# intel/intel-extension-for-transformers

Hardware: AMD Instinct MI355X
Metric: decode tokens/sec + achieved HBM GB/s, Llama-2-7B int4 WOQ, batch=1 (higher is better)
Workload: dtype int4 weights x fp32 activations (3 int8 limbs on i8 MFMA, exact int32 tile sums, fp32 across tiles); 1 GPU; Llama-2-7B int4 sym group_size=128 fp16 scales, batch=1 greedy decode, prompt 32, lm_head fp16 unquantised, KV fp16; global_batch=1, parallelism=single GPU, hipgraph=True

## Files before the change

include/woq_hip_experimental.h:

```cpp
#ifndef WOQ_HIP_EXPERIMENTAL_H_
#define WOQ_HIP_EXPERIMENTAL_H_

#include "woq_hip.h"

#ifdef __cplusplus
extern "C" {
#endif

WOQ_API int woq_engine_set_attn_chunk(woq_engine* e, int chunk);
WOQ_API int woq_engine_attn_chunk(woq_engine* e);
WOQ_API int woq_engine_time_gemv(woq_engine* e, int reps, void* stream, float* total_ms, double* bytes_per_pass,
                                 int* launches_per_pass);
WOQ_API int woq_engine_time_gemv_mask(woq_engine* e, int mask, int reps, void* stream, float* total_ms,
                                      double* bytes_per_pass, int* launches_per_pass);
WOQ_API int woq_engine_time_twin(woq_engine* e, int mode, int reps, void* stream, float* total_ms);
WOQ_API int woq_engine_set_time_eager(woq_engine* e, int on);
WOQ_API int woq_engine_time_prefill_gemm(woq_engine* e, int layer, int n_rows, int reps, void* stream, float* gemm_ms,
                                         float* call_ms);
WOQ_API int woq_gemm_form_log(int* forms, int cap);
WOQ_API int woq_probe_rope_append(void* qkv, int n_seq, int T, int start, int heads, int kv_heads, int head_dim,
                                  const float* cos_dev, const float* sin_dev, void* kcache, void* vcache, int kv_dtype,
                                  size_t seq_stride_elems, void* stream);
WOQ_API int woq_probe_attn_prefill(const void* qkv, int n_seq, int T, int start, int heads, int kv_heads, int head_dim,
                                   const void* kcache, const void* vcache, int kv_dtype, size_t seq_stride_elems,
                                   void* out, int window, void* stream);
WOQ_API int woq_probe_attn_decode(const float* qkv, void* kcache, void* vcache, int kv_dtype, const int32_t* pos_dev,
                                  const float* cos_dev, const float* sin_dev, int heads, int kv_heads, int head_dim,
                                  int max_ctx, int window, int splits, int grouped, int merge, int chunk_fixed,
                                  float* out, void* stream);
WOQ_API int woq_probe_sample(const float* logits, int vocab, uint32_t* seen, const woq_sampler_config* cfg,
                             const float* u_or_null, const int32_t* pos_dev, int32_t* token_out, uint32_t* philox_out4,
                             int* status, void* stream);

#ifdef __cplusplus
}
#endif
#endif
```

intel_extension_for_transformers_amd/_lib.py:

```python
import ctypes
import os

_HERE = os.path.dirname(os.path.abspath(__file__))
LIB_PATH = os.environ.get("WOQ_HIP_LIB") or os.path.join(_HERE, "libwoq_hip.so")

F32, BF16, F16, FP8_E4M3 = 0, 1, 2, 3
W_INT4_CLIP, W_INT8, W_NF4, W_FP4_E2M1, W_FP4_E2M1_BNB, W_INT3_CLIP, W_INT2_CLIP = 0, 1, 2, 3, 4, 5, 6
W_FP8_E4M3, W_FP8_E5M2 = 7, 8
S_FP8_E8M0 = 4
FLAG_SCALE_E8M0 = 4
C_FP32, C_BF16, C_INT8, C_FP16 = 0, 1, 2, 3
HEADER_BYTES = 256

WEIGHT_TYPES = {"int4_clip": W_INT4_CLIP, "int4": W_INT4_CLIP, "int8": W_INT8, "nf4": W_NF4, "fp4_e2m1": W_FP4_E2M1,
                "fp4": W_FP4_E2M1, "fp4_e2m1_bnb": W_FP4_E2M1_BNB, "int3_clip": W_INT3_CLIP, "int2_clip": W_INT2_CLIP,
                "fp8_e4m3": W_FP8_E4M3, "fp8": W_FP8_E4M3, "fp8_e5m2": W_FP8_E5M2}
SCALE_TYPES = {"fp32": F32, "bf16": BF16, "fp16": F16, "fp8_e8m0": S_FP8_E8M0}
COMPUTE_TYPES = {"fp32": C_FP32, "bf16": C_BF16, "int8": C_INT8, "fp16": C_FP16}
SCALE_NAMES = {F32: "fp32", BF16: "bf16", F16: "fp16"}
COMPUTE_NAMES = {v: k for k, v in COMPUTE_TYPES.items()}
WEIGHT_NAMES = {W_INT4_CLIP: "int4_clip", W_INT8: "int8", W_NF4: "nf4", W_FP4_E2M1: "fp4_e2m1",
                W_FP4_E2M1_BNB: "fp4_e2m1_bnb", W_FP8_E4M3: "fp8_e4m3", W_FP8_E5M2: "fp8_e5m2"}


class BlobHeader(ctypes.Structure):

    _fields_ = [
        ("magic", ctypes.c_uint32), ("version", ctypes.c_uint32), ("total_bytes", ctypes.c_uint64),
        ("K", ctypes.c_int32), ("N", ctypes.c_int32), ("group", ctypes.c_int32), ("Kpad", ctypes.c_int32),
        ("Npad", ctypes.c_int32), ("n_groups", ctypes.c_int32),
        ("weight_type", ctypes.c_uint32), ("scale_type", ctypes.c_uint32), ("compute_type", ctypes.c_uint32),
        ("flags", ctypes.c_uint32), ("scale_mode", ctypes.c_uint32), ("narrow_bits", ctypes.c_uint32),
        ("off_q", ctypes.c_uint64), ("off_scale", ctypes.c_uint64), ("off_zp", ctypes.c_uint64),
        ("off_shuffle", ctypes.c_uint64), ("pad", ctypes.c_uint8 * (HEADER_BYTES - 96)),
    ]


assert ctypes.sizeof(BlobHeader) == HEADER_BYTES


class EngineConfig(ctypes.Structure):
    _fields_ = [(n, ctypes.c_int32) for n in ("hidden", "inter", "heads", "kv_heads", "head_dim", "layers", "vocab",
                                              "max_ctx")] + [("rms_eps", ctypes.c_float), ("rope_theta", ctypes.c_float),
                                                             ("tp_rank", ctypes.c_int32), ("tp_size", ctypes.c_int32),
                                                             ("kv_dtype", ctypes.c_int32),
                                                             ("reserved", ctypes.c_int32 * 3)]


class LayerWeights(ctypes.Structure):
    _fields_ = [("qkv_blob", ctypes.c_void_p), ("o_blob", ctypes.c_void_p), ("gate_up_blob", ctypes.c_void_p),
                ("down_blob", ctypes.c_void_p), ("ln1", ctypes.c_void_p), ("ln2", ctypes.c_void_p),
                ("qkv_hdr", BlobHeader), ("o_hdr", BlobHeader), ("gate_up_hdr", BlobHeader), ("down_hdr", BlobHeader)]


class SamplerConfig(ctypes.Structure):

    _fields_ = [("do_sample", ctypes.c_int32), ("top_k", ctypes.c_int32), ("temperature", ctypes.c_float),
                ("top_p", ctypes.c_float), ("repetition_penalty", ctypes.c_float), ("seed_lo", ctypes.c_uint32),
                ("seed_hi", ctypes.c_uint32), ("reserved", ctypes.c_uint32)]


ALLREDUCE_FN = ctypes.CFUNCTYPE(ctypes.c_int, ctypes.c_void_p, ctypes.c_void_p, ctypes.c_size_t, ctypes.c_void_p)

EXPORTS = [
    "woq_last_error", "woq_abi_version", "woq_device_count", "woq_packed_weight_size",
    "woq_repack_quantized_weight", "woq_quantize_to_packed_weight", "woq_dequantize_packed_weight",
    "woq_read_header", "woq_blob_extract", "woq_linear", "woq_rmsnorm", "woq_rope", "woq_silu_mul", "woq_gelu",
    "woq_engine_create", "woq_engine_destroy", "woq_engine_set_layer", "woq_engine_set_head",
    "woq_engine_bind_io", "woq_engine_token_ptr", "woq_engine_pos_ptr", "woq_engine_logits_ptr", "woq_engine_hidden_ptr",
    "woq_engine_step", "woq_engine_capture", "woq_engine_replay", "woq_engine_steps", "woq_engine_set_allreduce",
    "woq_engine_phase", "woq_engine_prefill", "woq_engine_prefill_logits_ptr", "woq_engine_kv_cache_ptr",
    "woq_engine_set_attn_splits", "woq_engine_attn_splits", "woq_engine_set_attn_grouped", "woq_engine_attn_grouped",
    "woq_engine_set_tp_options", "woq_engine_set_fuse_attn", "woq_engine_fuse_attn", "woq_engine_status",
    "woq_engine_clear_status", "woq_comm_create", "woq_comm_handle", "woq_comm_connect", "woq_comm_allreduce_f32",
    "woq_comm_status", "woq_comm_set_timeout_ms", "woq_comm_destroy", "woq_engine_set_comm", "woq_set_workspace",
    "woq_engine_uses_xq", "woq_engine_token_log_ptr", "woq_table_digit_planes",
    "woq_engine_set_sampler", "woq_engine_sampler_seen", "woq_engine_sampler_seen_ptr",
]
EXPERIMENTAL_EXPORTS = [
    "woq_engine_set_attn_chunk", "woq_engine_attn_chunk", "woq_engine_time_gemv", "woq_engine_time_gemv_mask",
    "woq_engine_time_twin", "woq_engine_set_time_eager", "woq_engine_time_prefill_gemm", "woq_gemm_form_log",
    "woq_probe_rope_append", "woq_probe_attn_prefill", "woq_probe_attn_decode", "woq_probe_sample",
]
GEMM_FORM_FRAG, GEMM_FORM_SPLITK, GEMM_FORM_FP32, GEMM_FORM_HANDSCHED = 1, 2, 4, 8
GEMM_FORM_RING, GEMM_FORM_TALL, GEMM_FORM_RAW = 16, 32, 64

_lib = None


def lib():
    global _lib
    if _lib is not None:
        return _lib
    if not os.path.exists(LIB_PATH):
        raise RuntimeError(
            "QBits: %s not found. Build it with `python -c 'import __graft_entry__ as g; g.build()'` "
            "(hipcc --offload-arch=gfx950); there is no CPU fallback for the MI355X path." % LIB_PATH)
    L = ctypes.CDLL(LIB_PATH)
    vp, ci, cs, cf = ctypes.c_void_p, ctypes.c_int, ctypes.c_size_t, ctypes.c_float
    L.woq_last_error.restype = ctypes.c_char_p
    L.woq_packed_weight_size.restype = cs
    L.woq_packed_weight_size.argtypes = [ci] * 7
    L.woq_table_digit_planes.restype = ci
    L.woq_table_digit_planes.argtypes = [ci, ci, vp, vp]
    L.woq_repack_quantized_weight.argtypes = [vp, vp, vp, vp, ci, ci, ci, ci, ci, ci, vp, cs, vp]
    L.woq_quantize_to_packed_weight.argtypes = [vp, ci, ci, ci, ci, ci, ci, ci, ci, vp, cs, vp]
    L.woq_dequantize_packed_weight.argtypes = [vp, ctypes.POINTER(BlobHeader), vp, ci, vp]
    L.woq_read_header.argtypes = [vp, ctypes.POINTER(BlobHeader), vp]
    L.woq_blob_extract.argtypes = [vp, ctypes.POINTER(BlobHeader), ci, vp, vp]
    L.woq_linear.argtypes = [vp, ci, ci, vp, ctypes.POINTER(BlobHeader), vp, vp, ci, ci, ci, vp]
    L.woq_rmsnorm.argtypes = [vp, ci, vp, cf, ci, ci, vp, ci, vp]
    L.woq_rope.argtypes = [vp, ci, vp, vp, vp, ci, ci, ci, vp]
    L.woq_silu_mul.argtypes = [vp, vp, ci, cs, vp, vp]
    L.woq_gelu.argtypes = [vp, ci, cs, ci, vp, vp]
    L.woq_engine_create.argtypes = [ctypes.POINTER(EngineConfig), ctypes.POINTER(vp)]
    L.woq_engine_destroy.argtypes = [vp]
    L.woq_engine_destroy.restype = None
    L.woq_engine_set_layer.argtypes = [vp, ci, ctypes.POINTER(LayerWeights)]
    L.woq_engine_set_head.argtypes = [vp, vp, ci, vp, vp, ci, vp, vp]
    for f in ("woq_engine_token_ptr", "woq_engine_pos_ptr", "woq_engine_logits_ptr", "woq_engine_hidden_ptr"):
        getattr(L, f).restype = vp
        getattr(L, f).argtypes = [vp]
    L.woq_engine_bind_io.argtypes = [vp, vp, vp, vp, vp]
    L.woq_engine_step.argtypes = [vp, ci, vp]
    L.woq_engine_capture.argtypes = [vp, ci, vp]
    L.woq_engine_replay.argtypes = [vp, ci, vp]
    L.woq_engine_steps.argtypes = [vp, ci, ci, vp]
    L.woq_engine_set_time_eager.argtypes = [vp, ci]
    L.woq_engine_set_allreduce.argtypes = [vp, ALLREDUCE_FN, vp]
    L.woq_engine_phase.argtypes = [vp, ci, ci, ci, vp]
    L.woq_engine_prefill.argtypes = [vp, vp, ci, ci, ci, ci, vp]
    L.woq_engine_prefill_logits_ptr.restype = vp
    L.woq_engine_prefill_logits_ptr.argtypes = [vp]
    L.woq_engine_set_attn_splits.argtypes = [vp, ci]
    L.woq_engine_attn_splits.argtypes = [vp]
    L.woq_engine_set_attn_grouped.argtypes = [vp, ci]
    L.woq_engine_attn_grouped.argtypes = [vp]
    L.woq_engine_set_attn_chunk.argtypes = [vp, ci]
    L.woq_engine_attn_chunk.argtypes = [vp]
    L.woq_engine_set_fuse_attn.argtypes = [vp, ci]
    L.woq_engine_fuse_attn.argtypes = [vp]
    L.woq_engine_status.argtypes = [vp, vp]
    L.woq_engine_clear_status.argtypes = [vp, vp]
    L.woq_engine_kv_cache_ptr.restype = vp
    L.woq_engine_kv_cache_ptr.argtypes = [vp, ci]
    L.woq_engine_time_gemv.argtypes = [vp, ci, vp, ctypes.POINTER(cf), ctypes.POINTER(ctypes.c_double),
                                       ctypes.POINTER(ci)]
    L.woq_engine_time_gemv_mask.argtypes = [vp, ci, ci, vp, ctypes.POINTER(cf), ctypes.POINTER(ctypes.c_double),
                                            ctypes.POINTER(ci)]
    L.woq_engine_time_twin.argtypes = [vp, ci, ci, vp, ctypes.POINTER(cf)]
    L.woq_engine_set_tp_options.argtypes = [vp, ci, ci]
    L.woq_engine_time_prefill_gemm.argtypes = [vp, ci, ci, ci, vp, ctypes.POINTER(cf), ctypes.POINTER(cf)]
    L.woq_gemm_form_log.argtypes = [ctypes.POINTER(ci), ci]
    L.woq_probe_rope_append.argtypes = [vp, ci, ci, ci, ci, ci, ci, vp, vp, vp, vp, ci, cs, vp]
    L.woq_probe_attn_prefill.argtypes = [vp, ci, ci, ci, ci, ci, ci, vp, vp, ci, cs, vp, ci, vp]
    L.woq_probe_attn_decode.argtypes = [vp, vp, vp, ci, vp, vp, vp] + [ci] * 9 + [vp, vp]
    L.woq_comm_create.argtypes = [ci, ci, cs, ctypes.POINTER(vp)]
    L.woq_comm_handle.argtypes = [vp, vp, cs]
    L.woq_comm_connect.argtypes = [vp, vp, ctypes.POINTER(ci)]
    L.woq_comm_allreduce_f32.argtypes = [vp, vp, cs, vp]
    L.woq_comm_status.argtypes = [vp, vp, ctypes.POINTER(ci)]
    L.woq_comm_set_timeout_ms.argtypes = [vp, ci]
    L.woq_comm_destroy.argtypes = [vp]
    L.woq_comm_destroy.restype = None
    L.woq_engine_set_comm.argtypes = [vp, vp, ci]
    L.woq_set_workspace.argtypes = [vp, cs]
    L.woq_engine_uses_xq.argtypes = [vp]
    L.woq_engine_token_log_ptr.restype = vp
    L.woq_engine_token_log_ptr.argtypes = [vp]
    L.woq_engine_set_sampler.argtypes = [vp, ctypes.POINTER(SamplerConfig)]
    L.woq_engine_sampler_seen.argtypes = [vp, vp, ci, ci, vp]
    L.woq_engine_sampler_seen_ptr.restype = vp
    L.woq_engine_sampler_seen_ptr.argtypes = [vp]
    L.woq_probe_sample.argtypes = [vp, ci, vp, ctypes.POINTER(SamplerConfig), vp, vp, vp, vp, vp, vp]
    _lib = L
    return L


def gemm_form_log():
    buf = (ctypes.c_int * 64)()
    n = lib().woq_gemm_form_log(buf, 64)
    return list(buf[:min(n, 64)])


def _ptr(t):
    return ctypes.c_void_p(t.data_ptr())


def probe_rope_append(qkv, n_seq, T, start, heads, kv_heads, head_dim, cos, sin, kcache, vcache, kv_dtype, seq_stride):
    rc = lib().woq_probe_rope_append(_ptr(qkv), n_seq, T, start, heads, kv_heads, head_dim, _ptr(cos), _ptr(sin),
                                     _ptr(kcache), _ptr(vcache), kv_dtype, seq_stride, stream_ptr())
    if rc != 0:
        raise RuntimeError(lib().woq_last_error().decode())


def probe_attn_prefill(qkv, n_seq, T, start, heads, kv_heads, head_dim, kcache, vcache, kv_dtype, seq_stride, out,
                       window):
    rc = lib().woq_probe_attn_prefill(_ptr(qkv), n_seq, T, start, heads, kv_heads, head_dim, _ptr(kcache), _ptr(vcache),
                                      kv_dtype, seq_stride, _ptr(out), window, stream_ptr())
    if rc != 0:
        raise RuntimeError(lib().woq_last_error().decode())


def probe_attn_decode(qkv, kcache, vcache, kv_dtype, pos, cos, sin, heads, kv_heads, head_dim, max_ctx, window, splits,
                      grouped, merge, chunk_fixed, out):
    rc = lib().woq_probe_attn_decode(_ptr(qkv), _ptr(kcache), _ptr(vcache), kv_dtype, _ptr(pos), _ptr(cos), _ptr(sin),
                                     heads, kv_heads, head_dim, max_ctx, window, splits, grouped, merge, chunk_fixed,
                                     _ptr(out), stream_ptr())
    if rc != 0:
        raise RuntimeError(lib().woq_last_error().decode())


def sampler_config(do_sample=False, temperature=1.0, top_k=0, top_p=1.0, repetition_penalty=1.0, seed=0):
    seed = int(seed) & 0xFFFFFFFFFFFFFFFF
    return SamplerConfig(do_sample=int(bool(do_sample)), top_k=int(top_k or 0),
                         temperature=float(1.0 if temperature is None else temperature),
                         top_p=float(1.0 if top_p is None else top_p),
                         repetition_penalty=float(1.0 if repetition_penalty is None else repetition_penalty),
                         seed_lo=seed & 0xFFFFFFFF, seed_hi=seed >> 32, reserved=0)


def probe_sample(logits, seen, cfg, pos, token_out, u=None, philox_out=None, status=None):
    opt = lambda t: _ptr(t) if t is not None else None
    rc = lib().woq_probe_sample(_ptr(logits), int(logits.numel()), _ptr(seen), ctypes.byref(cfg), opt(u), _ptr(pos),
                                _ptr(token_out), opt(philox_out), opt(status), stream_ptr())
    if rc != 0:
        raise RuntimeError(lib().woq_last_error().decode())


def check(rc):
    if rc != 0:
        raise RuntimeError(lib().woq_last_error().decode())


def require_gpu():
    import torch

    if not torch.cuda.is_available() or lib().woq_device_count() == 0:
        raise RuntimeError("QBits: no MI355X/HIP device visible; the gfx950 WOQ path has no CPU fallback")


def torch_dtype_code(dt):
    import torch

    if dt == torch.float32:
        return F32
    if dt == torch.bfloat16:
        return BF16
    if dt == torch.float16:
        return F16
    raise RuntimeError("QBits: unsupported qbits data type.")


def stream_ptr():
    import torch

    return ctypes.c_void_p(torch.cuda.current_stream().cuda_stream)
```

intel_extension_for_transformers_amd/csrc/woq_host.h:

```cpp
#pragma once
#include "woq_comm_dev.h"
#include "woq_launch.h"
#include "woq_xq.h"

namespace woq {
struct AttnA2A;
struct AttnMerge;
struct LutArgs;

int launch_gemv_from_header(const void* act, int act_dtype, int lda, const void* blob, const woq_blob_header& h,
                            const float* bias, void* out, int out_dtype, int ldo, int M, const float* norm_w,
                            float eps, const float* residual, int ld_res, int epi, int nt, hipStream_t st);
int launch_gemv_fp8(const void* act, int act_dtype, int lda, const void* hi_blob, const woq_blob_header& hi,
                    const void* lo_q, uint32_t fp8_type, const float* bias, void* out, int out_dtype, int ldo, int M,
                    hipStream_t st);
int launch_gemv_fp8_engine(const float* act, int lda, const void* hi_blob, const woq_blob_header& hi, const void* lo_q,
                           uint32_t fp8_type, float* out, int ldo, const float* norm_w, float eps, const float* residual,
                           int ld_res, int epi, float* gu_tmp, hipStream_t st);

int lut_args_for(uint32_t weight_type, uint32_t compute_type, LutArgs& L);
bool gemv_tile_geometry(int tiles_k, int cb, int smode, int& nw, int& tpw);
int gemv_tile_k_chunks(int tiles_k, int cb, int smode, bool chainable);
int gemv_tile_max_rows(const void* act, int act_dtype, int lda, const woq_blob_header& h, const float* norm_w,
                       int epi, int out_dtype);
int launch_gemv_tile(const void* act, int act_dtype, int lda, int M, const void* blob, const woq_blob_header& h,
                     const float* bias, void* out, int out_dtype, int ldo, const float* norm_w, float eps,
                     const float* residual, int ld_res, int epi, hipStream_t st);

bool gemv_fp8_mfma_supported(const void* act, int act_dtype, int lda, const woq_blob_header& hi);
int launch_gemv_fp8_mfma(const void* act, int act_dtype, int lda, int M, const void* hi_blob, const woq_blob_header& hi,
                         const void* lo_q, uint32_t fp8_type, const float* bias, void* out, int out_dtype, int ldo,
                         hipStream_t st, const float* norm_w = nullptr, float eps = 0.f, const float* residual = nullptr,
                         int ld_res = 0);
void launch_silu_mul_tiles(const float* gu, int inter, float* act, hipStream_t st);

bool gemv_xq_supported(const woq_blob_header& h, int epi);
int launch_gemv_xq(const XqPtrs& xin, const void* blob, const woq_blob_header& h, const float* bias, float* out,
                   const float* ssq_in, float eps, const float* residual, int epi, const XqPtrs& xo,
                   const float* next_norm_w, float* ssq_out, hipStream_t st, const CommDev* tp);
int launch_gemv_twin(const void* blob, const woq_blob_header& h, int epi, int mode, unsigned int* sink, hipStream_t st);

bool gemv_xq_attn_supported(const woq_blob_header& h, int heads, int kv_heads, int head_dim, int kv_dtype, int max_ctx,
                            int window, int splits);
int launch_gemv_xq_attn(const XqPtrs& xin, const void* blob, const woq_blob_header& h, unsigned long long* qkv_g,
                        const float* ssq_in, float eps, const unsigned int* seq, int layer, int* status, void* kcache,
                        void* vcache, int kv_dtype, const int32_t* pos, const float* cs, const float* sn, int heads,
                        int kv_heads, int max_ctx, int window, float* attn_out, const XqPtrs& xq_attn, hipStream_t st,
                        int splits = 1, unsigned long long* part_g = nullptr);

void launch_embed(const void* embed, int dtype, const int32_t* token, int hidden, float* out, const float* norm_w,
                  const XqPtrs& xo, float* ssq_out, unsigned int* step_seq, int32_t* pos, int max_ctx, int* status,
                  hipStream_t st);
int launch_attn_decode(const float* qkv, void* kcache, void* vcache, int kv_dtype, const int32_t* pos,
                       const float* cs, const float* sn, int heads, int kv_heads, int D, int max_ctx, int window,
                       float* out, int splits, int grouped, float* part, const XqPtrs& xo, hipStream_t st,
                       unsigned int* merge_counters, int chunk_fixed, const AttnA2A* a2a_grouped = nullptr,
                       const unsigned int* seq = nullptr, int layer = 0);
void launch_attn_combine(const float* part, int heads, int D, int splits, float* out, const XqPtrs& xo,
                         hipStream_t st);
void launch_lm_head(const float* hidden_in, const float* norm_w, float eps, const void* W, int w_dtype, int hidden,
                    int vocab, float* logits, float* pmax, int32_t* pidx, hipStream_t st);
void launch_argmax(const float* logits, int vocab, int32_t* token, int32_t* pos, hipStream_t st);
void launch_argmax_pairs(const float* pmax, const int32_t* pidx, int n, int32_t* token, int32_t* pos, int32_t* log,
                         hipStream_t st);
void launch_argmax_embed(const float* pmax, const int32_t* pidx, int n, int32_t* token, int32_t* pos, int32_t* log,
                         const void* embed, int dtype, int hidden, float* out, const float* norm_w, const XqPtrs& xo,
                         float* ssq_out, unsigned int* step_seq, int max_ctx, int* status, hipStream_t st);

void launch_sample(const float* logits, int vocab, uint32_t* seen, const woq_sampler_config* cfg_dev, const float* u_dev,
                   int32_t* token, int32_t* pos_advance, const int32_t* pos_fixed, int32_t* log, uint32_t* philox_out,
                   int* status, hipStream_t st);
void launch_sampler_seen(uint32_t* seen, int vocab, const int32_t* tokens, int n, hipStream_t st);
void launch_sampler_config_store(const woq_sampler_config& cfg, woq_sampler_config* dst, hipStream_t st);
const char* sampler_config_problem(const woq_sampler_config& cfg);

void launch_embed_rows(const void* embed, int dtype, const int32_t* tokens, int M, int hidden, float* out,
                       hipStream_t st);
int launch_rope_append(_Float16* qkv, int n_seq, int T, int start, int heads, int kv_heads, int HD, const float* cs,
                       const float* sn, void* kcache, void* vcache, int kv_dtype, size_t seq_stride_elems,
                       hipStream_t st);
int launch_attn_prefill(const _Float16* qkv, int n_seq, int T, int start, int heads, int kv_heads, int HD,
                        const void* kcache, const void* vcache, int kv_dtype, size_t seq_stride_elems, _Float16* out,
                        int window, hipStream_t st);
void launch_gather_last(const float* h, int n_seq, int T, int hidden, float* dst, hipStream_t st);
bool launch_attn_decode_mfma(const float* qkv, void* kcache, void* vcache, int kv_dtype, const int32_t* pos,
                             const float* cs, const float* sn, int heads, int kv_heads, int D, int window, int splits,
                             float* part, int chunk_fixed, int max_ctx, const AttnMerge& mg, hipStream_t st);
int attn_decode_mfma_slots(int kv_dtype, int rep);

size_t gemm_f16_workspace_bytes_blob(int M, const woq_blob_header& h, int planes);
int launch_gemm_f16(const void* act, int act_dtype, int lda, const void* blob, const woq_blob_header& h,
                    const float* bias, void* out, int out_dtype, int ldo, int M, const float* norm_w, float eps,
                    const float* residual, int ld_res, int epi, void* ws, int fp32_class, hipStream_t st,
                    const void* fp8_lo = nullptr, uint32_t fp8_type = 0, size_t ws_bytes = 0);
void set_gemm_time_events(hipEvent_t before, hipEvent_t after);
}

size_t woq_comm_max_elems(woq_comm* c);
int woq_comm_launch_allreduce(woq_comm* c, float* buf, size_t n, hipStream_t st);
int woq_comm_launch_allreduce_ex(woq_comm* c, float* buf, size_t n, int pushed, const float* norm_w,
                                 const woq::XqPtrs& xo, float* ssq_out, hipStream_t st);
const woq::CommDev* woq_comm_dev_ptr(woq_comm* c);
int woq_comm_launch_greedy(woq_comm* c, const float* pmax, const int32_t* pidx, int n, int vocab_offset,
                           int32_t* token, int32_t* pos, int32_t* log, hipStream_t st);
```

intel_extension_for_transformers_amd/csrc/woq_ops.hip:

```cpp
#include "woq_attn_decode.h"
#include "woq_device.h"
#include "woq_host.h"
#include "woq_xq.h"
#include "../../include/woq_hip_experimental.h"

namespace woq {

__global__ __launch_bounds__(256) void rmsnorm_kernel(const void* __restrict__ x, int dtype,
                                                      const float* __restrict__ w, float eps, int d,
                                                      void* __restrict__ out, int out_dtype) {
  __shared__ float part[4];
  const size_t row = blockIdx.x;
  const int tid = threadIdx.x;
  float ss = 0.f;
  for (int i = tid; i < d; i += 256) {
    float v = load_f32(x, row * d + i, dtype);
    ss = fmaf(v, v, ss);
  }
  ss = wave_sum(ss);
  if ((tid & 63) == 0) part[tid >> 6] = ss;
  __syncthreads();
  const float tot = part[0] + part[1] + part[2] + part[3];
  const float inv = 1.0f / sqrtf(tot / (float)d + eps);
  for (int i = tid; i < d; i += 256) {
    float v = load_f32(x, row * d + i, dtype);
    store_f32(out, row * d + i, out_dtype, v * inv * w[i]);
  }
}

__global__ void rope_kernel(void* __restrict__ x, int dtype, const int32_t* __restrict__ pos,
                            const float* __restrict__ cs, const float* __restrict__ sn, int heads, int D,
                            size_t total_pairs) {
  size_t idx = (size_t)blockIdx.x * blockDim.x + threadIdx.x;
  if (idx >= total_pairs) return;
  const int half = D >> 1;
  const int i = (int)(idx % half);
  const size_t th = idx / half;
  const int t = (int)(th / heads);
  const int p = pos[t];
  const float c = cs[(size_t)p * half + i], s = sn[(size_t)p * half + i];
  const size_t base = th * D;
  const float a = load_f32(x, base + i, dtype), b = load_f32(x, base + i + half, dtype);
  store_f32(x, base + i, dtype, a * c - b * s);
  store_f32(x, base + i + half, dtype, b * c + a * s);
}

__global__ void silu_mul_kernel(const void* __restrict__ g, const void* __restrict__ u, int dtype, size_t n,
                                void* __restrict__ out) {
  size_t idx = (size_t)blockIdx.x * blockDim.x + threadIdx.x;
  const size_t stride = (size_t)gridDim.x * blockDim.x;
  for (; idx < n; idx += stride) {
    const float a = load_f32(g, idx, dtype), b = load_f32(u, idx, dtype);
    store_f32(out, idx, dtype, a / (1.0f + expf(-a)) * b);
  }
}

__global__ void gelu_kernel(const void* __restrict__ x, int dtype, size_t n, int approximate,
                            void* __restrict__ out) {
  size_t idx = (size_t)blockIdx.x * blockDim.x + threadIdx.x;
  const size_t stride = (size_t)gridDim.x * blockDim.x;
  for (; idx < n; idx += stride) {
    const float v = load_f32(x, idx, dtype);
    float r;
    if (approximate)
      r = 0.5f * v * (1.0f + tanhf(0.7978845608028654f * (v + 0.044715f * v * v * v)));
    else
      r = 0.5f * v * (1.0f + erff(v * 0.7071067811865476f));
    store_f32(out, idx, dtype, r);
  }
}


__global__ void embed_kernel(const void* __restrict__ embed, int dtype, const int32_t* __restrict__ token, int hidden,
                             float* __restrict__ out, const float* __restrict__ norm_w, XqPtrs xo,
                             float* __restrict__ ssq_out, unsigned int* __restrict__ step_seq,
                             int32_t* __restrict__ pos, int max_ctx, int* __restrict__ status) {
  const int i = blockIdx.x * blockDim.x + threadIdx.x;
  if (i == 0) {
    if (step_seq != nullptr) step_seq[0] = step_seq[0] + 1u;
    if (pos != nullptr && pos[0] >= max_ctx) {
      pos[0] = max_ctx - 1;
      if (status != nullptr) atomicOr(status, 2);
    }
  }
  if (i < hidden) {
    const float v = load_f32(embed, (size_t)token[0] * hidden + i, dtype);
    out[i] = v;
    if (xo.limbs != nullptr) {
      const float ss = row16_sum(v * v);
      if ((i & 15) == 0) ssq_out[i >> 4] = ss;
      xq_emit16(v * norm_w[i], xo, i >> 4, i & 15);
    }
  }
}

__global__ __launch_bounds__(256) void argmax_embed_kernel(const float* __restrict__ pmax, const int32_t* __restrict__ pidx,
                                                           int n_pairs, int32_t* __restrict__ token,
                                                           int32_t* __restrict__ pos, int32_t* __restrict__ log,
                                                           const void* __restrict__ embed, int dtype, int hidden,
                                                           float* __restrict__ out, const float* __restrict__ norm_w,
                                                           XqPtrs xo, float* __restrict__ ssq_out,
                                                           unsigned int* __restrict__ step_seq, int max_ctx,
                                                           int* __restrict__ status) {
  __shared__ float bv[4];
  __shared__ int bi[4];
  const int tid = threadIdx.x, lane = tid & 63, wid = tid >> 6;
  float best = -INFINITY;
  int idx = 0x7fffffff;
  for (int i = tid; i < n_pairs; i += 256) {
    const float v = pmax[i];
    const int ci = pidx[i];
    if (v > best || (v == best && ci < idx)) best = v, idx = ci;
  }
#pragma unroll
  for (int o = 32; o > 0; o >>= 1) {
    const float ov = __shfl_xor(best, o, 64);
    const int oi = __shfl_xor(idx, o, 64);
    if (ov > best || (ov == best && oi < idx)) best = ov, idx = oi;
  }
  if (lane == 0) bv[wid] = best, bi[wid] = idx;
  __syncthreads();
  best = bv[0], idx = bi[0];
#pragma unroll
  for (int w = 1; w < 4; ++w)
    if (bv[w] > best || (bv[w] == best && bi[w] < idx)) best = bv[w], idx = bi[w];
  const bool no_winner = idx < 0 || (size_t)idx >= (size_t)n_pairs * 16;
  if (no_winner) idx = 0;
  if (blockIdx.x == 0 && tid == 0) {
    if (no_winner && status != nullptr) atomicOr(status, 4);
    token[0] = idx;
    int p = pos[0];
    if (log != nullptr) log[p] = idx;
    p += 1;
    if (step_seq != nullptr) step_seq[0] = step_seq[0] + 1u;
    if (p >= max_ctx) {
      p = max_ctx - 1;
      if (status != nullptr) atomicOr(status, 2);
    }
    pos[0] = p;
  }
  const int i = blockIdx.x * 256 + tid;
  if (i < hidden) {
    const float v = load_f32(embed, (size_t)idx * hidden + i, dtype);
    out[i] = v;
    if (xo.limbs != nullptr) {
      const float ss = row16_sum(v * v);
      if ((i & 15) == 0) ssq_out[i >> 4] = ss;
      xq_emit16(v * norm_w[i], xo, i >> 4, i & 15);
    }
  }
}

template <typename KV, int HD, bool SPLIT>
__global__ __launch_bounds__(256) void attn_decode_kernel(const float* __restrict__ qkv, KV* __restrict__ kcache,
                                                          KV* __restrict__ vcache, const int32_t* __restrict__ pos_p,
                                                          const float* __restrict__ cs, const float* __restrict__ sn,
                                                          int hk, int window, int spw,
                                                          float* __restrict__ out, XqPtrs xo, AttnMerge mg) {
  extern __shared__ __attribute__((aligned(16))) float sm[];
  const int heads = hk & 0xffff, kv_heads = hk >> 16;
  const int bx = (int)blockIdx.x;
  const int h = (heads & 7) == 0 ? (bx & 7) * (heads >> 3) + (bx >> 3) : bx;
  attn_decode_body<KV, HD, SPLIT>(sm, h, (int)blockIdx.y, (int)gridDim.y, AttnPlain{qkv}, kcache, vcache, pos_p, cs,
                                  sn, heads, kv_heads, window, spw, out, xo);
  if constexpr (SPLIT) {
    if (mg.counter != nullptr) attn_slices_merge<HD, 1>(out, heads, h, 1, (int)gridDim.y, mg.counter + h, mg, sm);
  }
}

template <int HD>
__global__ __launch_bounds__(256) void attn_combine_kernel(const float* __restrict__ part, int ns,
                                                          float* __restrict__ out, XqPtrs xo) {
  __shared__ float ms[64], wl[64], wsc[64], red[256];
  constexpr int GROUPS = 256 / HD;
  constexpr int PER = ATTN_MAX_SLICES / GROUPS;
  const int h = blockIdx.x, tid = threadIdx.x;
  const int d = tid % HD, grp = tid / HD;
  const float* p = part + (size_t)h * ATTN_MAX_SLICES * HD;
  const float* pml = part + (size_t)gridDim.x * ATTN_MAX_SLICES * HD + (size_t)h * ATTN_MAX_SLICES * 2;
  const int si = min(tid, ns - 1);
  const float m_r = pml[si * 2], l_r = pml[si * 2 + 1];
  float v[PER];
#pragma unroll
  for (int u = 0; u < PER; ++u) v[u] = p[(size_t)min(grp + u * GROUPS, ns - 1) * HD + d];
  if (tid < ns) ms[tid] = m_r, wl[tid] = l_r;
  __syncthreads();
  float m = -INFINITY;
  for (int s = 0; s < ns; ++s) m = fmaxf(m, ms[s]);
  if (tid < ns) {
    const float w = ms[tid] == -INFINITY ? 0.f : __expf(ms[tid] - m);
    wsc[tid] = w;
    wl[tid] *= w;
  }
  __syncthreads();
  float l = 0.f;
  for (int s = 0; s < ns; ++s) l += wl[s];
  float o = 0.f;
#pragma unroll
  for (int u = 0; u < PER; ++u) {
    const int s = grp + u * GROUPS;
    if (s < ns) o = fmaf(v[u], wsc[s], o);
  }
  red[tid] = o;
  __syncthreads();
  if (grp == 0) {
    float t = 0.f;
#pragma unroll
    for (int g2 = 0; g2 < GROUPS; ++g2) t += red[g2 * HD + d];
    out[(size_t)h * HD + d] = t / l;
    if (xo.limbs != nullptr) xq_emit16(t / l, xo, (h * HD + d) >> 4, d & 15);
  }
}

__global__ __launch_bounds__(256) void lm_head_kernel(const float* __restrict__ hidden_in,
                                                      const float* __restrict__ norm_w, float eps,
                                                      const void* __restrict__ W, int w_dtype, int hidden, int vocab,
                                                      float* __restrict__ logits, float* __restrict__ pmax,
                                                      int32_t* __restrict__ pidx) {
  extern __shared__ __attribute__((aligned(16))) float sm[];
  float* xs = sm;
  __shared__ float part[4];
  __shared__ float bestv[4];
  __shared__ int besti[4];
  const int tid = threadIdx.x, lane = tid & 63, wid = tid >> 6;
  float wbest = -INFINITY;
  int wbi = 0x7fffffff;
  typedef unsigned int u32x4 __attribute__((ext_vector_type(4)));
  float ss = 0.f;
  for (int i = tid; i < hidden; i += 256) {
    const float v = hidden_in[i];
    xs[i] = v;
    ss = fmaf(v, v, ss);
  }
  ss = wave_sum(ss);
  if (lane == 0) part[wid] = ss;
  __syncthreads();
  const float inv = 1.0f / sqrtf((part[0] + part[1] + part[2] + part[3]) / (float)hidden + eps);
  for (int i = tid; i < hidden; i += 256) xs[i] = xs[i] * inv * norm_w[i];
  __syncthreads();
  const int rows_per_wg = 16;
  auto consume = [&](const u32x4& raw, int k0, float& acc) {
    const uint32_t rr[4] = {raw.x, raw.y, raw.z, raw.w};
#pragma unroll
    for (int j = 0; j < 4; ++j) {
      float lo, hi;
      if (w_dtype == WOQ_BF16) {
        lo = bf16_bits_to_f32(rr[j] & 0xffff);
        hi = bf16_bits_to_f32(rr[j] >> 16);
      } else {
        lo = f16_bits_to_f32(rr[j] & 0xffff);
        hi = f16_bits_to_f32(rr[j] >> 16);
      }
      acc = fmaf(lo, xs[k0 + 2 * j], acc);
      acc = fmaf(hi, xs[k0 + 2 * j + 1], acc);
    }
  };
  auto finish = [&](int v, float acc) {
    acc = wave_sum(acc);
    if (lane == 0) logits[v] = acc;
    if (acc > wbest) {
      wbest = acc;
      wbi = v;
    }
  };
  for (int r = wid; r < rows_per_wg; r += 4) {
    const int v = blockIdx.x * rows_per_wg + r;
    if (v >= vocab) break;
    const uint16_t* wr = (const uint16_t*)W + (size_t)v * hidden;
    float acc = 0.f;
    for (int k0 = lane * 8; k0 < hidden; k0 += 512) consume(__builtin_nontemporal_load((const u32x4*)(wr + k0)), k0, acc);
    finish(v, acc);
  }
  if (pmax) {
    if (lane == 0) {
      bestv[wid] = wbest;
      besti[wid] = wbi;
    }
    __syncthreads();
    if (tid == 0) {
      float b = bestv[0];
      int bi = besti[0];
      for (int w = 1; w < 4; ++w)
        if (bestv[w] > b || (bestv[w] == b && besti[w] < bi)) {
          b = bestv[w];
          bi = besti[w];
        }
      pmax[blockIdx.x] = b;
      pidx[blockIdx.x] = bi;
    }
  }
}

__global__ __launch_bounds__(1024) void argmax_kernel(const float* __restrict__ logits, const int32_t* __restrict__ cand,
                                                      int vocab, int32_t* __restrict__ token,
                                                      int32_t* __restrict__ pos, int32_t* __restrict__ log) {
  __shared__ float bv[16];
  __shared__ int bi[16];
  const int tid = threadIdx.x, lane = tid & 63, wid = tid >> 6;
  float best = -INFINITY;
  int idx = 0x7fffffff;
  for (int i = tid; i < vocab; i += 1024) {
    const float v = logits[i];
    const int ci = cand ? cand[i] : i;
    if (v > best || (v == best && ci < idx)) {
      best = v;
      idx = ci;
    }
  }
#pragma unroll
  for (int o = 32; o > 0; o >>= 1) {
    const float ov = __shfl_xor(best, o, 64);
    const int oi = __shfl_xor(idx, o, 64);
    if (ov > best || (ov == best && oi < idx)) {
      best = ov;
      idx = oi;
    }
  }
  if (lane == 0) {
    bv[wid] = best;
    bi[wid] = idx;
  }
  __syncthreads();
  if (tid == 0) {
    for (int w = 1; w < 16; ++w)
      if (bv[w] > best || (bv[w] == best && bi[w] < idx)) {
        best = bv[w];
        idx = bi[w];
      }
    token[0] = idx;
    if (log != nullptr) log[pos[0]] = idx;
    pos[0] = pos[0] + 1;
  }
}

void launch_embed(const void* embed, int dtype, const int32_t* token, int hidden, float* out, const float* norm_w,
                  const XqPtrs& xo, float* ssq_out, unsigned int* step_seq, int32_t* pos, int max_ctx, int* status,
                  hipStream_t st) {
  hipLaunchKernelGGL(embed_kernel, dim3((hidden + 255) / 256), dim3(256), 0, st, embed, dtype, token, hidden, out,
                     norm_w, xo, ssq_out, step_seq, pos, max_ctx, status);
}

template <typename KV, int HD>
static int launch_attn_t(const float* qkv, void* kcache, void* vcache, const int32_t* pos, const float* cs,
                         const float* sn, int heads, int kv_heads, int max_ctx, int window, float* out, int splits,
                         float* part, const XqPtrs& xo, unsigned int* merge_counters, hipStream_t st) {
  const int reach = window > 0 ? min(window, max_ctx) : max_ctx;
  const int span = splits > 1 ? ((((reach + splits - 1) / splits) + 63) & ~63) + 64 : reach;
  const int spw = attn_dec_spw(span);
  const size_t lds = attn_dec_lds_floats(HD, span) * 4;
  if (lds > 160 * 1024) return woq::fail("QBits: max_ctx too large for the decode attention (raise attn_splits)");
  if (splits > 1) {
    auto k = attn_decode_kernel<KV, HD, true>;
    static bool once = false;
    if (!once) {
      hipFuncSetAttribute((const void*)k, hipFuncAttributeMaxDynamicSharedMemorySize, 160 * 1024);
      once = true;
    }
    const AttnMerge mg{merge_counters, out, xo};
    hipLaunchKernelGGL(k, dim3(heads, splits), dim3(256), lds, st, qkv, (KV*)kcache, (KV*)vcache, pos, cs, sn,
                       heads | (kv_heads << 16), window, spw, part, XqPtrs{nullptr, nullptr, nullptr}, mg);
    if (merge_counters == nullptr)
      hipLaunchKernelGGL(attn_combine_kernel<HD>, dim3(heads), dim3(256), 0, st, part, splits, out, xo);
    return 0;
  }
  auto k = attn_decode_kernel<KV, HD, false>;
  static bool once = false;
  if (!once) {
    hipFuncSetAttribute((const void*)k, hipFuncAttributeMaxDynamicSharedMemorySize, 160 * 1024);
    once = true;
  }
  hipLaunchKernelGGL(k, dim3(heads), dim3(256), lds, st, qkv, (KV*)kcache, (KV*)vcache, pos, cs, sn,
                     heads | (kv_heads << 16), window, spw, out, xo,
                     AttnMerge{nullptr, nullptr, XqPtrs{nullptr, nullptr, nullptr}});
  return 0;
}

int launch_attn_decode(const float* qkv, void* kcache, void* vcache, int kv_dtype, const int32_t* pos,
                       const float* cs, const float* sn, int heads, int kv_heads, int D, int max_ctx, int window,
                       float* out, int splits, int grouped, float* part, const XqPtrs& xo, hipStream_t st,
                       unsigned int* merge_counters, int chunk_fixed, const AttnA2A* a2a_grouped, const unsigned int* seq,
                       int layer) {
  if (D != 64 && D != 128) return woq::fail("QBits: attention head_dim must be 64 or 128");
  if (splits > ATTN_MAX_SLICES) return woq::fail("QBits: at most 64 context slices");
  AttnMerge mg{merge_counters, out, xo};
  const bool a2a = grouped && a2a_grouped != nullptr && merge_counters == nullptr && splits <= 32;
  if (a2a) mg.part_g = a2a_grouped->part_g, mg.seq = seq, mg.layer = layer, mg.status = a2a_grouped->status;
  if (grouped && launch_attn_decode_mfma(qkv, kcache, vcache, kv_dtype, pos, cs, sn, heads, kv_heads, D, window, splits,
                                          part, chunk_fixed, max_ctx, mg, st)) {
    if (merge_counters == nullptr && !a2a) launch_attn_combine(part, heads, D, splits, out, xo, st);
    return 0;
  }
#define WOQ_ATTN_DEC(T)                                                                                              \
  return D == 128 ? launch_attn_t<T, 128>(qkv, kcache, vcache, pos, cs, sn, heads, kv_heads, max_ctx, window, out,   \
                                          splits, part, xo, merge_counters, st)                                     \
                  : launch_attn_t<T, 64>(qkv, kcache, vcache, pos, cs, sn, heads, kv_heads, max_ctx, window, out,    \
                                         splits, part, xo, merge_counters, st);
  if (kv_dtype == WOQ_F16) { WOQ_ATTN_DEC(_Float16) }
  if (kv_dtype == WOQ_FP8_E4M3) { WOQ_ATTN_DEC(Fp8) }
  WOQ_ATTN_DEC(__bf16)
#undef WOQ_ATTN_DEC
}

void launch_attn_combine(const float* part, int heads, int D, int splits, float* out, const XqPtrs& xo,
                         hipStream_t st) {
  if (D == 128)
    hipLaunchKernelGGL(attn_combine_kernel<128>, dim3(heads), dim3(256), 0, st, part, splits, out, xo);
  else
    hipLaunchKernelGGL(attn_combine_kernel<64>, dim3(heads), dim3(256), 0, st, part, splits, out, xo);
}

void launch_lm_head(const float* hidden_in, const float* norm_w, float eps, const void* W, int w_dtype, int hidden,
                    int vocab, float* logits, float* pmax, int32_t* pidx, hipStream_t st) {
  hipLaunchKernelGGL(lm_head_kernel, dim3((vocab + 15) / 16), dim3(256), (size_t)hidden * 4, st, hidden_in, norm_w,
                     eps, W, w_dtype, hidden, vocab, logits, pmax, pidx);
}

void launch_argmax(const float* logits, int vocab, int32_t* token, int32_t* pos, hipStream_t st) {
  hipLaunchKernelGGL(argmax_kernel, dim3(1), dim3(1024), 0, st, logits, (const int32_t*)nullptr, vocab, token, pos,
                     (int32_t*)nullptr);
}

void launch_argmax_pairs(const float* pmax, const int32_t* pidx, int n, int32_t* token, int32_t* pos, int32_t* log,
                         hipStream_t st) {
  hipLaunchKernelGGL(argmax_kernel, dim3(1), dim3(1024), 0, st, pmax, pidx, n, token, pos, log);
}

void launch_argmax_embed(const float* pmax, const int32_t* pidx, int n, int32_t* token, int32_t* pos, int32_t* log,
                         const void* embed, int dtype, int hidden, float* out, const float* norm_w, const XqPtrs& xo,
                         float* ssq_out, unsigned int* step_seq, int max_ctx, int* status, hipStream_t st) {
  hipLaunchKernelGGL(argmax_embed_kernel, dim3((hidden + 255) / 256), dim3(256), 0, st, pmax, pidx, n, token, pos, log,
                     embed, dtype, hidden, out, norm_w, xo, ssq_out, step_seq, max_ctx, status);
}

}

using namespace woq;

extern "C" {

int woq_rmsnorm(const void* x_dev, int dtype, const float* weight_dev, float eps, int rows, int d, void* out_dev,
                int out_dtype, void* stream) {
  WOQ_TRY
  WOQ_CHECK(rows >= 0 && d > 0, "QBits: bad rmsnorm shape");
  if (rows == 0) return 0;
  hipLaunchKernelGGL(rmsnorm_kernel, dim3(rows), dim3(256), 0, (hipStream_t)stream, x_dev, dtype, weight_dev, eps, d,
                     out_dev, out_dtype);
  WOQ_HIP(hipGetLastError());
  WOQ_END
}

int woq_rope(void* x_dev, int dtype, const int32_t* pos_dev, const float* cos_dev, const float* sin_dev, int tokens,
             int heads, int D, void* stream) {
  WOQ_TRY
  WOQ_CHECK((D & 1) == 0, "QBits: rope head_dim must be even");
  size_t total = (size_t)tokens * heads * (D / 2);
  if (total == 0) return 0;
  hipLaunchKernelGGL(rope_kernel, dim3((unsigned)((total + 255) / 256)), dim3(256), 0, (hipStream_t)stream, x_dev,
                     dtype, pos_dev, cos_dev, sin_dev, heads, D, total);
  WOQ_HIP(hipGetLastError());
  WOQ_END
}

int woq_silu_mul(const void* gate_dev, const void* up_dev, int dtype, size_t n, void* out_dev, void* stream) {
  WOQ_TRY
  if (n == 0) return 0;
  unsigned blocks = (unsigned)std::min<size_t>((n + 255) / 256, 2048);
  hipLaunchKernelGGL(silu_mul_kernel, dim3(blocks), dim3(256), 0, (hipStream_t)stream, gate_dev, up_dev, dtype, n,
                     out_dev);
  WOQ_HIP(hipGetLastError());
  WOQ_END
}

int woq_gelu(const void* x_dev, int dtype, size_t n, int approximate, void* out_dev, void* stream) {
  WOQ_TRY
  if (n == 0) return 0;
  unsigned blocks = (unsigned)std::min<size_t>((n + 255) / 256, 2048);
  hipLaunchKernelGGL(gelu_kernel, dim3(blocks), dim3(256), 0, (hipStream_t)stream, x_dev, dtype, n, approximate,
                     out_dev);
  WOQ_HIP(hipGetLastError());
  WOQ_END
}

WOQ_API int woq_probe_attn_decode(const float* qkv, void* kcache, void* vcache, int kv_dtype, const int32_t* pos_dev,
                                  const float* cos_dev, const float* sin_dev, int heads, int kv_heads, int head_dim,
                                  int max_ctx, int window, int splits, int grouped, int merge, int chunk_fixed,
                                  float* out, void* stream) {
  WOQ_TRY
  WOQ_CHECK(heads > 0 && kv_heads > 0 && heads % kv_heads == 0 && max_ctx > 0 && window >= 0 && splits >= 1,
            "QBits: bad attention shape");
  WOQ_CHECK(merge == 0 || merge == 1, "QBits: merge must be 0 (combine launch) or 1 (last-arriver counters)");
  const hipStream_t st = (hipStream_t)stream;
  const size_t part_bytes = (size_t)heads * ATTN_MAX_SLICES * (head_dim + 2) * sizeof(float);
  float* part = nullptr;
  unsigned int* counters = nullptr;
  WOQ_HIP(hipMallocAsync((void**)&part, part_bytes, st));
  if (merge) {
    if (hipMallocAsync((void**)&counters, (size_t)heads * sizeof(unsigned int), st) != hipSuccess ||
        hipMemsetAsync(counters, 0, (size_t)heads * sizeof(unsigned int), st) != hipSuccess) {
      if (counters) hipFreeAsync(counters, st);
      hipFreeAsync(part, st);
      return woq::fail("QBits: could not allocate the attention merge counters");
    }
  }
  const int rc = launch_attn_decode(qkv, kcache, vcache, kv_dtype, pos_dev, cos_dev, sin_dev, heads, kv_heads, head_dim,
                                    max_ctx, window, out, splits, grouped, part, XqPtrs{nullptr, nullptr, nullptr}, st,
                                    counters, chunk_fixed, nullptr, nullptr, 0);
  const hipError_t le = hipGetLastError();
  if (counters) hipFreeAsync(counters, st);
  hipFreeAsync(part, st);
  if (rc) return rc;
  WOQ_HIP(le);
  WOQ_END
}

}
```

Baseline: 693.6 tokens/s.

## Add streamed lm_head kernel with double-buffered nontemporal row loads

Adds a templated lm_head kernel for fixed hidden sizes. Each wave streams one fp16 or bf16 vocab row at a time using 128-bit nontemporal loads, double-buffering the next row while the current one is multiplied. RMSNorm is fused into the block prologue and reduced with permlane/DPP wave sums, and the kernel keeps the per-block argmax pair output. It is dispatched by default for hidden 4096, and a probe API can force the generic or streamed form; the cost is extra specialised code paths and fixed launch bounds/occupancy per shape.

```diff
diff --git a/include/woq_hip_experimental.h b/include/woq_hip_experimental.h
--- a/include/woq_hip_experimental.h
+++ b/include/woq_hip_experimental.h
@@ -31,6 +31,8 @@
 WOQ_API int woq_probe_sample(const float* logits, int vocab, uint32_t* seen, const woq_sampler_config* cfg,
                              const float* u_or_null, const int32_t* pos_dev, int32_t* token_out, uint32_t* philox_out4,
                              int* status, void* stream);
+WOQ_API int woq_probe_lm_head(const float* hidden_in, const float* norm_w, float eps, const void* W, int w_dtype,
+                              int hidden, int vocab, float* logits, float* pmax, int32_t* pidx, int form, void* stream);
 
 #ifdef __cplusplus
 }
diff --git a/intel_extension_for_transformers_amd/_lib.py b/intel_extension_for_transformers_amd/_lib.py
--- a/intel_extension_for_transformers_amd/_lib.py
+++ b/intel_extension_for_transformers_amd/_lib.py
@@ -81,6 +81,7 @@
     "woq_engine_set_attn_chunk", "woq_engine_attn_chunk", "woq_engine_time_gemv", "woq_engine_time_gemv_mask",
     "woq_engine_time_twin", "woq_engine_set_time_eager", "woq_engine_time_prefill_gemm", "woq_gemm_form_log",
     "woq_probe_rope_append", "woq_probe_attn_prefill", "woq_probe_attn_decode", "woq_probe_sample",
+    "woq_probe_lm_head",
 ]
 GEMM_FORM_FRAG, GEMM_FORM_SPLITK, GEMM_FORM_FP32, GEMM_FORM_HANDSCHED = 1, 2, 4, 8
 GEMM_FORM_RING, GEMM_FORM_TALL, GEMM_FORM_RAW = 16, 32, 64
@@ -173,6 +174,7 @@
     L.woq_engine_sampler_seen_ptr.restype = vp
     L.woq_engine_sampler_seen_ptr.argtypes = [vp]
     L.woq_probe_sample.argtypes = [vp, ci, vp, ctypes.POINTER(SamplerConfig), vp, vp, vp, vp, vp, vp]
+    L.woq_probe_lm_head.argtypes = [vp, vp, cf, vp, ci, ci, ci, vp, vp, vp, ci, vp]
     _lib = L
     return L
 
@@ -228,6 +230,17 @@
         raise RuntimeError(lib().woq_last_error().decode())
 
 
+LM_HEAD_DISPATCH, LM_HEAD_GENERIC, LM_HEAD_STREAM = 0, 1, 2
+
+
+def probe_lm_head(hidden_in, norm_w, eps, W, hidden, vocab, logits, pmax=None, pidx=None, form=LM_HEAD_DISPATCH):
+    opt = lambda t: _ptr(t) if t is not None else None
+    rc = lib().woq_probe_lm_head(_ptr(hidden_in), _ptr(norm_w), eps, _ptr(W), torch_dtype_code(W.dtype), hidden, vocab,
+                                 _ptr(logits), opt(pmax), opt(pidx), form, stream_ptr())
+    if rc != 0:
+        raise RuntimeError(lib().woq_last_error().decode())
+
+
 def check(rc):
     if rc != 0:
         raise RuntimeError(lib().woq_last_error().decode())
diff --git a/intel_extension_for_transformers_amd/csrc/woq_host.h b/intel_extension_for_transformers_amd/csrc/woq_host.h
--- a/intel_extension_for_transformers_amd/csrc/woq_host.h
+++ b/intel_extension_for_transformers_amd/csrc/woq_host.h
@@ -59,7 +59,7 @@
 void launch_attn_combine(const float* part, int heads, int D, int splits, float* out, const XqPtrs& xo,
                          hipStream_t st);
 void launch_lm_head(const float* hidden_in, const float* norm_w, float eps, const void* W, int w_dtype, int hidden,
-                    int vocab, float* logits, float* pmax, int32_t* pidx, hipStream_t st);
+                    int vocab, float* logits, float* pmax, int32_t* pidx, hipStream_t st, int form = 0);
 void launch_argmax(const float* logits, int vocab, int32_t* token, int32_t* pos, hipStream_t st);
 void launch_argmax_pairs(const float* pmax, const int32_t* pidx, int n, int32_t* token, int32_t* pos, int32_t* log,
                          hipStream_t st);
diff --git a/intel_extension_for_transformers_amd/csrc/woq_lm_head.h b/intel_extension_for_transformers_amd/csrc/woq_lm_head.h
--- /dev/null
+++ b/intel_extension_for_transformers_amd/csrc/woq_lm_head.h
@@ -0,0 +1,135 @@
+#pragma once
+#include "woq_device.h"
+
+namespace woq {
+
+__device__ __forceinline__ float wave_sum_xor_valu(float v) {
+  float a = v, b = v;
+  asm volatile("v_nop\n\tv_nop\n\tv_permlane32_swap_b32 %0, %1" : "+v"(a), "+v"(b));
+  v = a + b;
+  a = v, b = v;
+  asm volatile("v_nop\n\tv_nop\n\tv_permlane16_swap_b32 %0, %1" : "+v"(a), "+v"(b));
+  v = a + b;
+  v += WOQ_DPP_F32(v, 0x128);
+  v += WOQ_DPP_F32(v, 0x124);
+  v += WOQ_DPP_F32(v, 0x4E);
+  v += WOQ_DPP_F32(v, 0xB1);
+  return v;
+}
+
+constexpr bool lm_head_stream_shape(int hidden) {
+  return hidden == 512 || hidden == 1024 || hidden == 4096 || hidden == 8192;
+}
+
+template <int C, int U, int OCC, bool BF16, bool MATH>
+__global__ __launch_bounds__(256, OCC) void lm_head_stream_kernel(const float* __restrict__ hidden_in,
+                                                                  const float* __restrict__ norm_w, float eps,
+                                                                  const void* __restrict__ W, int hidden, int vocab,
+                                                                  float* __restrict__ logits, float* __restrict__ pmax,
+                                                                  int32_t* __restrict__ pidx) {
+  static_assert(C % U == 0, "a unit never straddles two rows");
+  constexpr int HID = 512 * C, XPT = HID / 256, UPR = C / U, NU = 4 * UPR;
+  typedef unsigned int u32x4 __attribute__((ext_vector_type(4)));
+  __shared__ __attribute__((aligned(16))) float xs[HID];
+  __shared__ float part[4];
+  __shared__ float bestv[4];
+  __shared__ int besti[4];
+  const int tid = threadIdx.x, lane = tid & 63, wid = tid >> 6;
+
+  float x[XPT], nw[XPT];
+#pragma unroll
+  for (int j = 0; j < XPT; ++j) x[j] = hidden_in[tid + 256 * j];
+#pragma unroll
+  for (int j = 0; j < XPT; ++j) nw[j] = norm_w[tid + 256 * j];
+
+  const int v0 = blockIdx.x * 16 + wid;
+  const uint16_t* wl = (const uint16_t*)W + lane * 8;
+  auto request = [&](u32x4 (&buf)[U], int n) {
+    const int v = min(v0 + 4 * (n / UPR), vocab - 1);
+    const u32x4* p = (const u32x4*)(wl + (size_t)v * HID + (n % UPR) * U * 512);
+#pragma unroll
+    for (int u = 0; u < U; ++u) buf[u] = __builtin_nontemporal_load(p + u * 64);
+  };
+  u32x4 buf[2][U];
+  request(buf[0], 0);
+  __builtin_amdgcn_sched_barrier(0);
+
+  float ss = 0.f;
+#pragma unroll
+  for (int j = 0; j < XPT; ++j) ss = fmaf(x[j], x[j], ss);
+  ss = wave_sum_xor_valu(ss);
+  if (lane == 0) part[wid] = ss;
+  __syncthreads();
+  const float inv = 1.0f / sqrtf((part[0] + part[1] + part[2] + part[3]) / (float)hidden + eps);
+#pragma unroll
+  for (int j = 0; j < XPT; ++j) xs[tid + 256 * j] = x[j] * inv * nw[j];
+  __syncthreads();
+
+  float wbest = -INFINITY;
+  int wbi = 0x7fffffff;
+  float acc = 0.f;
+#pragma unroll
+  for (int n = 0; n < NU; ++n) {
+    if (n + 1 < NU) request(buf[(n + 1) & 1], n + 1);
+    const u32x4(&cur)[U] = buf[n & 1];
+    if constexpr (MATH) {
+#pragma unroll
+      for (int u = 0; u < U; ++u) {
+        const int k0 = lane * 8 + ((n % UPR) * U + u) * 512;
+        const float4_t xa = *(const float4_t*)(xs + k0), xb = *(const float4_t*)(xs + k0 + 4);
+        const float xv[8] = {xa.x, xa.y, xa.z, xa.w, xb.x, xb.y, xb.z, xb.w};
+        const uint32_t rr[4] = {cur[u].x, cur[u].y, cur[u].z, cur[u].w};
+#pragma unroll
+        for (int j = 0; j < 4; ++j) {
+          float lo, hi;
+          if constexpr (BF16) {
+            lo = bf16_bits_to_f32(rr[j] & 0xffff);
+            hi = bf16_bits_to_f32(rr[j] >> 16);
+          } else {
+            lo = f16_bits_to_f32(rr[j] & 0xffff);
+            hi = f16_bits_to_f32(rr[j] >> 16);
+            asm("" : "+v"(lo));
+            asm("" : "+v"(hi));
+          }
+          acc = fmaf(lo, xv[2 * j], acc);
+          acc = fmaf(hi, xv[2 * j + 1], acc);
+        }
+      }
+    } else {
+#pragma unroll
+      for (int u = 0; u < U; ++u) asm volatile("" ::"v"(cur[u]));
+    }
+    if (n % UPR == UPR - 1) {
+      const int v = v0 + 4 * (n / UPR);
+      acc = wave_sum_xor_valu(acc);
+      if (v < vocab) {
+        if (lane == 0) logits[v] = acc;
+        if (acc > wbest) {
+          wbest = acc;
+          wbi = v;
+        }
+      }
+      acc = 0.f;
+    }
+  }
+  if (pmax) {
+    if (lane == 0) {
+      bestv[wid] = wbest;
+      besti[wid] = wbi;
+    }
+    __syncthreads();
+    if (tid == 0) {
+      float b = bestv[0];
+      int bi = besti[0];
+      for (int w = 1; w < 4; ++w)
+        if (bestv[w] > b || (bestv[w] == b && besti[w] < bi)) {
+          b = bestv[w];
+          bi = besti[w];
+        }
+      pmax[blockIdx.x] = b;
+      pidx[blockIdx.x] = bi;
+    }
+  }
+}
+
+}
diff --git a/intel_extension_for_transformers_amd/csrc/woq_ops.hip b/intel_extension_for_transformers_amd/csrc/woq_ops.hip
--- a/intel_extension_for_transformers_amd/csrc/woq_ops.hip
+++ b/intel_extension_for_transformers_amd/csrc/woq_ops.hip
@@ -1,6 +1,7 @@
 #include "woq_attn_decode.h"
 #include "woq_device.h"
 #include "woq_host.h"
+#include "woq_lm_head.h"
 #include "woq_xq.h"
 #include "../../include/woq_hip_experimental.h"
 
@@ -409,8 +410,28 @@
     hipLaunchKernelGGL(attn_combine_kernel<64>, dim3(heads), dim3(256), 0, st, part, splits, out, xo);
 }
 
+template <int C, int U, int OCC>
+static void launch_lm_head_stream(const float* hidden_in, const float* norm_w, float eps, const void* W, int w_dtype,
+                                  int hidden, int vocab, float* logits, float* pmax, int32_t* pidx, hipStream_t st) {
+  if (w_dtype == WOQ_BF16)
+    hipLaunchKernelGGL((lm_head_stream_kernel<C, U, OCC, true, true>), dim3((vocab + 15) / 16), dim3(256), 0, st,
+                       hidden_in, norm_w, eps, W, hidden, vocab, logits, pmax, pidx);
+  else
+    hipLaunchKernelGGL((lm_head_stream_kernel<C, U, OCC, false, true>), dim3((vocab + 15) / 16), dim3(256), 0, st,
+                       hidden_in, norm_w, eps, W, hidden, vocab, logits, pmax, pidx);
+}
+
 void launch_lm_head(const float* hidden_in, const float* norm_w, float eps, const void* W, int w_dtype, int hidden,
-                    int vocab, float* logits, float* pmax, int32_t* pidx, hipStream_t st) {
+                    int vocab, float* logits, float* pmax, int32_t* pidx, hipStream_t st, int form) {
+#define WOQ_LM_STREAM(C, U, OCC)                                                                                   \
+  return launch_lm_head_stream<C, U, OCC>(hidden_in, norm_w, eps, W, w_dtype, hidden, vocab, logits, pmax, pidx, st)
+  if (form != 1 && vocab > 0) {
+    if (hidden == 4096) WOQ_LM_STREAM(8, 8, 4);
+    if (hidden == 8192) WOQ_LM_STREAM(16, 8, 2);
+    if (hidden == 1024) WOQ_LM_STREAM(2, 2, 4);
+    if (hidden == 512) WOQ_LM_STREAM(1, 1, 4);
+  }
+#undef WOQ_LM_STREAM
   hipLaunchKernelGGL(lm_head_kernel, dim3((vocab + 15) / 16), dim3(256), (size_t)hidden * 4, st, hidden_in, norm_w,
                      eps, W, w_dtype, hidden, vocab, logits, pmax, pidx);
 }
@@ -513,4 +534,18 @@
   WOQ_END
 }
 
-}
+WOQ_API int woq_probe_lm_head(const float* hidden_in, const float* norm_w, float eps, const void* W, int w_dtype,
+                              int hidden, int vocab, float* logits, float* pmax, int32_t* pidx, int form,
+                              void* stream) {
+  WOQ_TRY
+  WOQ_CHECK(hidden > 0 && vocab > 0, "QBits: bad lm_head shape");
+  WOQ_CHECK(w_dtype == WOQ_F16 || w_dtype == WOQ_BF16, "QBits: lm_head rows are fp16 or bf16");
+  WOQ_CHECK(form >= 0 && form <= 2, "QBits: lm_head form must be 0 (dispatch), 1 (generic) or 2 (streamed)");
+  WOQ_CHECK((pmax == nullptr) == (pidx == nullptr), "QBits: lm_head pairs come as both arrays or neither");
+  WOQ_CHECK(form != 2 || lm_head_stream_shape(hidden), "QBits: the streamed lm_head needs hidden 512, 1024, 4096 or 8192");
+  launch_lm_head(hidden_in, norm_w, eps, W, w_dtype, hidden, vocab, logits, pmax, pidx, (hipStream_t)stream, form);
+  WOQ_HIP(hipGetLastError());
+  WOQ_END
+}
+
+}
```

Result: no change. 695.6 tokens/s, median of 6 (+0.3%).
